# payakorn/InteriorPointMethod

Hardware: AMD Instinct MI355X
Metric: IPM iterations/sec (m=4096,n=8192 dense LP) (higher is better)
Workload: dtype f64; 1 GPU; dense synthetic LP m=4096 n=8192 fp64, seed 0, start x=s=1 y=0 (BASELINE.json configs[1]); replicas per GPU

## Files before the change

interiorpointmethod_amd/csrc/ipm_api.hip:

```cpp
#include <hip/hip_runtime.h>
#include <hip/hip_ext.h>
#include <math.h>
#include <stdarg.h>
#include <stdio.h>
#include <stdlib.h>
#include <string.h>

#include <deque>
#include <vector>

#include "../../include/ipm_hip.h"
#include "gemm_nt_f64.h"
#include "adat_syrk_f64.h"
#include "chol_update_f64.h"
#include "potrf_f64.h"
#include "sparse_ops.h"
#include "trsv_grouped.h"
#include "getrf_f64.h"
#include "small_lp.h"
#include "sparse_chol.h"
#include "sparse_symbolic.h"
#include "vector_ops.h"
#include "form_factor.h"
#include "lockstep.h"
#include "lockstep_merge.h"

#include <algorithm>
#include <atomic>
#include <mutex>
#include <chrono>
#include <limits>
#include <utility>

using namespace ipm;

static thread_local char g_err[512] = "";

static const int MAX_DEVICES = 64;
static std::atomic<int> g_live[MAX_DEVICES];
static std::atomic<bool> g_attr_set[MAX_DEVICES];

struct ipm_handle {
    int device = 0;
    hipStream_t stream = nullptr;
    bool own_stream = false;
    hipStream_t stream2 = nullptr;
    hipStream_t stream3 = nullptr;
    hipEvent_t ev_mid = nullptr, ev_res = nullptr, ev_grp = nullptr, ev_last = nullptr;
    std::vector<hipEvent_t> ev_diag, ev_crit, ev_bulk;
    hipEvent_t ev_fork = nullptr;
    int lookahead = 1;
    int grouped_trsv = 1;
    int gsz = 0;
    double *gXT = nullptr, *gX = nullptr, *gS = nullptr, *gPart = nullptr;
    unsigned* d_bulk_done = nullptr;
    bool no_dense = false;
    double* B_own = nullptr; double* invD_own = nullptr;
    int group_steps = 0;
    int two_level = 1;
    int bulk_variant = 0;
    int ss_small_blocks = 16;
    int flag_sync = 1;
    int last_gs = 1, n_counter_steps = 0, n_event_steps = 0, timeouts_recovered = 0;
    bool counted = false;
    bool small = false;
    int fused_small = 1;
    bool list_form = false;
    int list_form_opt = 1;
    int *ls_bi = nullptr, *ls_bk = nullptr;
    double* ls_bak = nullptr;
    int sm_nb = 0;
    int *sm_bptr = nullptr, *sm_bcol = nullptr;
    unsigned short *sm_bi = nullptr, *sm_bk = nullptr;
    double* sm_bcoef = nullptr;
    bool spf = false;
    bool spf_off = false;
    bool sp_serial = false;
    SpFactor spF;
    std::vector<void*> sp_allocs;
    int *sp_fptr = nullptr, *sp_fcol = nullptr;
    double* sp_fcoef = nullptr;
    long long* sp_diagpos = nullptr;
    long long sp_nslot = 0, sp_nu = 0, sp_terms = 0;
    int sp_height = 0, sp_rmax = 0, sp_grid = 1, sp_serial_launches = 0, sp_nvirtual = 0;
    size_t sp_lds_chol = 0, sp_lds_solve = 0;
    int sp_fv_off = 0;
    int sp_fuse_fwd = 1;
    const double* sp_fwd_fused = nullptr;
    int sp_lds_doubles = 16, sp_threads = 256;
    int sp_level_mode = 0;
    std::vector<int> sp_lvlptr;
    SpRec* sp_rec_level = nullptr;
    unsigned sp_epoch = 0;
    double shift_rel = 0.0;
    int auto_reg = 0;
    unsigned* d_flags = nullptr;
    int64_t m = 0, n = 0, mp = 0, np = 0;
    int nblk = 0, rc_chunks = 0, rows_per_chunk = 0, vblk = 0;
    ipm_options opt;
    void* ws = nullptr;
    size_t ws_bytes = 0;
    bool own_ws = false;
    double *A = nullptr, *B = nullptr, *invD = nullptr;
    double *x = nullptr, *s = nullptr, *c = nullptr, *rc = nullptr, *d = nullptr, *v = nullptr, *q = nullptr;
    double *dxa = nullptr, *dsa = nullptr, *dx = nullptr, *ds = nullptr;
    double *y = nullptr, *b = nullptr, *rb = nullptr, *t1 = nullptr, *t2 = nullptr, *dya = nullptr, *dy = nullptr;
    double *atp = nullptr, *part = nullptr, *slab = nullptr;
    int ff_enabled = 1;
    int ff_min_nblk = 16, ff_max_nblk = 72;
    bool ff_forced = false;
    int ff_chain_mode = 1;
    int ff_q = 4;
    int ff_workers = 0;
    int* d_ff_tile_items = nullptr;
    int ff_qmax = 16;
    bool ff_built = false, ff_last = false;
    FFSchedule ff_sched;
    FFItem* d_ff_items = nullptr;
    unsigned* d_ff_flags = nullptr;
    size_t ff_flag_words = 0;
    double* ff_slab = nullptr;
    double* ff_part = nullptr;
    hipEvent_t ev_ffjoin = nullptr;
    long long* ff_trace = nullptr;
    long long* ff_prof = nullptr;
    const int* fdone = nullptr;
    std::vector<int> env_last, env_first;
    bool use_env = false;
    int envelope = 1;
    bool sparse = false;
    int64_t nnz_cap = 0, nnz = 0;
    int* d_tile_order = nullptr;
    int *d_rowptr = nullptr, *d_colind = nullptr, *d_colptr = nullptr, *d_rowind = nullptr;
    double *d_rval = nullptr, *d_cval = nullptr;
    long long* stamp_buf = nullptr;
    unsigned* ff_potrfdone = nullptr;
    Scalars* sc = nullptr;
    IterRec* hist = nullptr;
    double* snap = nullptr;
    bool bnd = false;
    int bnd_nU = 0;
    double* bnd_mem = nullptr;
    bool detect = false;
    double det_eps_p = 1e-8, det_eps_d = 1e-8;
    double* det = nullptr;
    double* cert_mem = nullptr;
    int* fixed = nullptr;
    Scalars* h_sc = nullptr;
    bool haveA = false, haveBC = false, haveState = false, predictor_valid = false;
    bool fresh_state = true;
    int profiling = 0;
    double phase_ms[4] = {0, 0, 0, 0};
    hipEvent_t ev0 = nullptr, ev1 = nullptr;
// ... 280 lines not shown
    if (const char* e = getenv("IPM_ENVELOPE")) h->envelope = atoi(e);
    CREATE_TRY(hipMemsetAsync(base + L.off_inv, 0, L.off_slab - L.off_inv, h->stream));
    {
        std::lock_guard<std::mutex> lock(g_hsc_mutex);
        if (!g_hsc_pool.empty()) { h->h_sc = g_hsc_pool.back(); g_hsc_pool.pop_back(); }
    }
    if (!h->h_sc) CREATE_TRY(hipHostMalloc((void**)&h->h_sc, sizeof(Scalars), hipHostMallocDefault));
    memset(h->h_sc, 0, sizeof(Scalars));
    CREATE_TRY(hipEventCreate(&h->ev0));
    CREATE_TRY(hipEventCreate(&h->ev1));
    if (const char* e = getenv("IPM_LOOKAHEAD")) h->lookahead = atoi(e);
    h->detect = (h->opt.flags & IPM_FLAG_DETECT_INFEASIBILITY) != 0;
    if (h->opt.flags & IPM_FLAG_LOCKSTEP) { h->lockstep = 1; h->opt.flags |= IPM_FLAG_SINGLE_STREAM | IPM_FLAG_NO_DEVICE_POLLING; }
    if (h->opt.flags & IPM_FLAG_SINGLE_STREAM) h->lookahead = 0;
    if (const char* e = getenv("IPM_GROUPED_TRSV")) h->grouped_trsv = atoi(e);
    if (h->lockstep && getenv("IPM_LS_BLOCK_STEPS")) h->grouped_trsv = 0;
    if (h->lockstep) h->ss_small_blocks = 1 << 20;
    if (h->no_dense) h->grouped_trsv = 0;
    h->gsz = 0;
    if (h->grouped_trsv) {
        const bool ragged = !(getenv("IPM_RAGGED_GROUPS") && atoi(getenv("IPM_RAGGED_GROUPS")) == 0);
        if (h->nblk >= 2 * GS_MAX) { if (ragged || h->nblk % GS_MAX == 0) h->gsz = GS_MAX; }
        else {
            for (int p2 = GS_MAX; p2 >= 2; p2 /= 2) if (h->nblk % p2 == 0) { h->gsz = p2; break; }
            if (ragged && h->nblk > GS_MAX && h->gsz < 4) h->gsz = GS_MAX;
        }
    }
    if (h->gsz > 0) {
        const size_t nG = (size_t)h->nblk / h->gsz, GR = (size_t)h->gsz * 128;
        CREATE_TRY(dev_malloc(device, h->stream, (void**)&h->gXT, sizeof(double) * nG * GR * GR));
        CREATE_TRY(dev_malloc(device, h->stream, (void**)&h->gX, sizeof(double) * nG * GR * GR));
        CREATE_TRY(dev_malloc(device, h->stream, (void**)&h->gS, sizeof(double) * nG * (GR / 2) * (GR / 2)));
        CREATE_TRY(dev_malloc(device, h->stream, (void**)&h->gPart, sizeof(double) * 16 * (size_t)h->mp));
        CREATE_TRY(hipMemsetAsync(h->gXT, 0, sizeof(double) * nG * GR * GR, h->stream));
        CREATE_TRY(hipMemsetAsync(h->gX, 0, sizeof(double) * nG * GR * GR, h->stream));
    } else {
        h->grouped_trsv = 0;
    }
    CREATE_TRY(dev_malloc(device, h->stream, (void**)&h->d_flags, sizeof(unsigned) * (2 * (size_t)h->nblk + 4)));
    CREATE_TRY(hipMemsetAsync(h->d_flags, 0, sizeof(unsigned) * (2 * (size_t)h->nblk + 4), h->stream));
    CREATE_TRY(dev_malloc(device, h->stream, (void**)&h->d_bulk_done, sizeof(unsigned) * (2 * (size_t)h->nblk + 4)));
    CREATE_TRY(hipMemsetAsync(h->d_bulk_done, 0, sizeof(unsigned) * (2 * (size_t)h->nblk + 4), h->stream));
    if (const char* e = getenv("IPM_FLAG_SYNC")) h->flag_sync = atoi(e);
    if (h->opt.flags & IPM_FLAG_NO_DEVICE_POLLING) h->flag_sync = 0;
    if (const char* e = getenv("IPM_BULK_VARIANT")) h->bulk_variant = atoi(e);
    if (const char* e = getenv("IPM_TWO_LEVEL")) h->two_level = atoi(e);
    if (const char* e = getenv("IPM_GROUP_STEPS")) h->group_steps = atoi(e);
    if (const char* e = getenv("IPM_FUSED_SMALL")) h->fused_small = atoi(e);
    if (const char* e = getenv("IPM_LIST_FORM")) h->list_form_opt = atoi(e);
    if (getenv("IPM_POTRF_STAMPS")) { CREATE_TRY(dev_malloc(device, h->stream, (void**)&h->stamp_buf, 8 * 64 * sizeof(long long))); CREATE_TRY(hipMemsetAsync(h->stamp_buf, 0, 8 * 64 * sizeof(long long), h->stream)); }
    if (h->lookahead != 0 && h->nblk > 2)
        CREATE_TRY(hipStreamCreateWithFlags(&h->stream2, hipStreamNonBlocking));
    CREATE_TRY(hipEventCreateWithFlags(&h->ev_fork, hipEventDisableTiming));
    if (!h->sparse && h->lookahead != 0 && h->nblk >= 16)
        CREATE_TRY(hipStreamCreateWithFlags(&h->stream3, hipStreamNonBlocking));
    CREATE_TRY(hipEventCreateWithFlags(&h->ev_mid, hipEventDisableTiming));
    CREATE_TRY(hipEventCreateWithFlags(&h->ev_res, hipEventDisableTiming));
    CREATE_TRY(hipEventCreateWithFlags(&h->ev_grp, hipEventDisableTiming));
    CREATE_TRY(hipEventCreateWithFlags(&h->ev_last, hipEventDisableTiming));
    if (const char* e = getenv("IPM_FUSED_FACTOR")) { if (!strcmp(e, "force")) { h->ff_enabled = 1; h->ff_min_nblk = 3; h->ff_forced = true; } else h->ff_enabled = atoi(e); }
    if (const char* e = getenv("IPM_FF_MAX_NBLK")) h->ff_max_nblk = atoi(e);
    if (const char* e = getenv("IPM_FF_CHAIN_MODE")) {
        if (atoi(e) == 0) {
            int rc_ = fail(nullptr, IPM_ERR_INVALID_ARG, "IPM_FF_CHAIN_MODE=0 is not supported (the fused launch runs chain mode 1 only)");
            ipm_destroy(h);
            return rc_;
        }
    }
    if (const char* e = getenv("IPM_FF_Q")) h->ff_q = std::max(1, std::min(16, atoi(e)));
    CREATE_TRY(hipEventCreateWithFlags(&h->ev_ffjoin, hipEventDisableTiming));
    h->ev_diag.assign(h->nblk, nullptr); h->ev_crit.assign(h->nblk, nullptr); h->ev_bulk.assign(h->nblk, nullptr);
    for (int k = 0; k < h->nblk; ++k) {
        CREATE_TRY(hipEventCreateWithFlags(&h->ev_diag[k], hipEventDisableTiming));
        CREATE_TRY(hipEventCreateWithFlags(&h->ev_crit[k], hipEventDisableTiming));
        CREATE_TRY(hipEventCreateWithFlags(&h->ev_bulk[k], hipEventDisableTiming));
    }
    if (h->sparse && h->mp <= SP_LDS_MAX_MP && device < MAX_DEVICES && !g_attr_set[device].load(std::memory_order_acquire)) {
        CREATE_TRY(hipFuncSetAttribute((const void*)adat_sparse_kernel, hipFuncAttributeMaxDynamicSharedMemorySize, SP_LDS_MAX_MP * 8));
        g_attr_set[device].store(true, std::memory_order_release);
    }
    hipLaunchKernelGGL(set_params_kernel, dim3(1), dim3(1), 0, h->stream, h->sc, 1e-8, 1e-8, 1e-8, h->opt.eta, 5000, 0, 1);
    CREATE_TRY(hipGetLastError());
// ... 4 lines not shown
    return IPM_OK;
}

extern "C" int ipm_destroy(ipm_handle* h) {
    if (!h) return IPM_OK;
    (void)hipSetDevice(h->device);
    if (h->ff_prof) {
        (void)hipDeviceSynchronize();
        std::vector<long long> P(16 * ((size_t)h->ff_workers + 1));
        (void)hipMemcpy(P.data(), h->ff_prof, sizeof(long long) * P.size(), hipMemcpyDeviceToHost);
        double tot[16] = {0};
        for (int w = 0; w <= h->ff_workers; ++w) for (int k = 0; k < 16; ++k) tot[k] += (double)P[(size_t)w * 16 + k];
        static const char* nm[] = {"ticket", "F gemm", "F store+publish", "T wait", "T gemm", "T base+combine", "panel wait", "panel gemm", "T store+publish"};
        double sum = 0; for (int k = 0; k < 9; ++k) sum += tot[k];
        fprintf(stderr, "[ff prof] %d workers, F items %.0f, T items %.0f, cycles per worker in the launches %.3g (sum of phases %.3g)\n", h->ff_workers, tot[FFP_NF], tot[FFP_NT], tot[FFP_TOTAL] / h->ff_workers, sum / h->ff_workers);
        for (int k = 0; k < 9; ++k) fprintf(stderr, "   %-18s %6.2f %%\n", nm[k], 100.0 * tot[k] / sum);
    }
    if (h->counted) g_live[h->device].fetch_sub(1, std::memory_order_acq_rel);
    if (h->stream) (void)hipStreamSynchronize(h->stream);
    if (h->stream2) (void)hipStreamSynchronize(h->stream2);
    for (auto& v : {&h->ev_diag, &h->ev_crit, &h->ev_bulk})
        for (hipEvent_t e : *v) if (e) (void)hipEventDestroy(e);
    if (h->ev_fork) (void)hipEventDestroy(h->ev_fork);
    if (h->stream3) { (void)hipStreamSynchronize(h->stream3); (void)hipStreamDestroy(h->stream3); }
    if (h->ev_mid) (void)hipEventDestroy(h->ev_mid);
    if (h->ev_res) (void)hipEventDestroy(h->ev_res);
    if (h->ev_grp) (void)hipEventDestroy(h->ev_grp);
    if (h->ev_last) (void)hipEventDestroy(h->ev_last);
    if (h->ev_ffjoin) (void)hipEventDestroy(h->ev_ffjoin);
    if (h->stream2) (void)hipStreamDestroy(h->stream2);
    if (h->ev0) (void)hipEventDestroy(h->ev0);
    if (h->ev1) (void)hipEventDestroy(h->ev1);
    if (h->h_sc) { std::lock_guard<std::mutex> lock(g_hsc_mutex); g_hsc_pool.push_back(h->h_sc); h->h_sc = nullptr; }
    for (void* p : {(void*)h->stamp_buf, (void*)h->d_flags, (void*)h->d_bulk_done, (void*)h->B_own, (void*)h->invD_own, (void*)h->bnd_mem, (void*)h->cert_mem, (void*)h->gXT, (void*)h->gX, (void*)h->gS, (void*)h->gPart})
        dev_free(h->device, h->stream, p);
    ff_release(h);
    free_sparse_factor(h);
    for (void* p : {(void*)h->sm_bptr, (void*)h->sm_bcol, (void*)h->sm_bi, (void*)h->sm_bk, (void*)h->sm_bcoef, (void*)h->ls_bi, (void*)h->ls_bk, (void*)h->ls_bak})
        dev_free(h->device, h->stream, p);
    if (h->own_ws && h->ws) (void)hipFree(h->ws);
    if (h->own_stream && h->stream) (void)hipStreamDestroy(h->stream);
    delete h;
    return IPM_OK;
}

static bool all_finite(const double* p, int64_t rows, int64_t cols, int64_t ld) {
    for (int64_t i = 0; i < rows; ++i)
        for (int64_t j = 0; j < cols; ++j)
            if (!isfinite(p[i * ld + j])) return false;
    return true;
}

extern "C" int ipm_set_A_dense(ipm_handle* h, const double* A, int64_t ld, int is_device) {
    if (!h || !A || ld < h->n) return fail(h, IPM_ERR_INVALID_ARG, "ipm_set_A_dense: bad arguments");
    if (h->sparse) return fail(h, IPM_ERR_STATE, "ipm_set_A_dense: the handle was created for a sparse A (sparse_nnz > 0)");
    HIP_TRY(h, hipSetDevice(h->device));
    if (!is_device && !all_finite(A, h->m, h->n, ld)) return fail(h, IPM_ERR_INVALID_INPUT, "A has non-finite entries");
    HIP_TRY(h, hipMemsetAsync(h->A, 0, sizeof(double) * h->mp * h->np, h->stream));
    HIP_TRY(h, hipMemcpy2DAsync(h->A, sizeof(double) * h->np, A, sizeof(double) * ld, sizeof(double) * h->n, h->m,
                                is_device ? hipMemcpyDeviceToDevice : hipMemcpyHostToDevice, h->stream));
    HIP_TRY(h, hipStreamSynchronize(h->stream));
    h->haveA = true; h->predictor_valid = false;
    return IPM_OK;
}

static void free_sparse_factor(ipm_handle* h) {
    for (void* p : h->sp_allocs) dev_free(h->device, h->stream, p);
// ... 924 lines not shown
    h->ff_qmax = 1;
    for (int q_ : h->ff_sched.tile_q) h->ff_qmax = std::max(h->ff_qmax, q_);
    if (nstages > 65535) return fail(h, IPM_ERR_INVALID_ARG, "fused factor: %d formation stages exceed the 16-bit stage range of a work item", nstages);
    const size_t ntile = (size_t)h->nblk * (h->nblk + 1) / 2;
    {
        std::vector<int> fcnt(ntile, 0), base(ntile, 0), applied(ntile, 0), paneled(ntile, 0);
        for (const FFItem& it : h->ff_sched.items) {
            const size_t t = (size_t)ff_tile(it.i, it.c);
            if (it.type == FF_D) continue;
            if (it.type == FF_F) {
                if (it.c <= it.i) fcnt[t]++;
                if (it.i + 1 < h->nblk) fcnt[(size_t)ff_tile(it.i + 1, it.c)]++;
                continue;
            }
            if (it.t.j0 != applied[t]) return fail(h, IPM_ERR_INVALID_ARG, "fused factor: internal error (column order of tile %d,%d)", it.i, it.c);
            applied[t] = it.t.j1;
            if (it.t.flags & FF_ADD_BASE) base[t]++;
            if (it.t.flags & FF_PANEL) paneled[t]++;
        }
        for (int i = 0; i < h->nblk; ++i)
            for (int c = 0; c <= i; ++c) {
                const size_t t = (size_t)ff_tile(i, c);
                if (fcnt[t] != h->ff_sched.tile_q[t] || base[t] != 1 || applied[t] != ff_limit(i, c) || paneled[t] != (ff_needs_panel(i, c) ? 1 : 0))
                    return fail(h, IPM_ERR_INVALID_ARG, "fused factor: internal error (tile %d,%d incomplete in the work list)", i, c);
            }
    }
    const size_t nit = h->ff_sched.items.size();
    HIP_TRY(h, dev_malloc(h->device, h->stream, (void**)&h->d_ff_items, sizeof(FFItem) * nit));
    HIP_TRY(h, hipMemcpyAsync(h->d_ff_items, h->ff_sched.items.data(), sizeof(FFItem) * nit, hipMemcpyHostToDevice, h->stream));
    HIP_TRY(h, dev_malloc(h->device, h->stream, (void**)&h->d_ff_tile_items, sizeof(int) * 2 * ntile));
    HIP_TRY(h, hipMemcpyAsync(h->d_ff_tile_items, h->ff_sched.tile_items.data(), sizeof(int) * ntile, hipMemcpyHostToDevice, h->stream));
    HIP_TRY(h, hipMemcpyAsync(h->d_ff_tile_items + ntile, h->ff_sched.tile_q.data(), sizeof(int) * ntile, hipMemcpyHostToDevice, h->stream));
    h->ff_flag_words = 32 + 2 * ntile + 3 * (size_t)h->nblk;
    HIP_TRY(h, dev_malloc(h->device, h->stream, (void**)&h->d_ff_flags, sizeof(unsigned) * 2 * h->ff_flag_words));
    HIP_TRY(h, dev_malloc(h->device, h->stream, (void**)&h->ff_slab, sizeof(double) * ntile * (size_t)h->ff_qmax * 128 * 128));
    HIP_TRY(h, dev_malloc(h->device, h->stream, (void**)&h->ff_part, sizeof(double) * 256));
    if (getenv("IPM_FF_PROF")) {
        HIP_TRY(h, dev_malloc(h->device, h->stream, (void**)&h->ff_prof, sizeof(long long) * 16 * ((size_t)h->ff_workers + 1)));
        HIP_TRY(h, hipMemsetAsync(h->ff_prof, 0, sizeof(long long) * 16 * ((size_t)h->ff_workers + 1), h->stream));
    }
    if (getenv("IPM_FF_TRACE_ITEMS")) {
        const size_t words = 4 * nit + 12 * (size_t)h->nblk;
        HIP_TRY(h, dev_malloc(h->device, h->stream, (void**)&h->ff_trace, sizeof(long long) * words));
        HIP_TRY(h, hipMemsetAsync(h->ff_trace, 0, sizeof(long long) * words, h->stream));
    }
    HIP_TRY(h, hipStreamSynchronize(h->stream));
    h->ff_built = true;
    return IPM_OK;
}

static void ff_release(ipm_handle* h) {
    for (void** p : {(void**)&h->d_ff_items, (void**)&h->d_ff_flags, (void**)&h->ff_slab, (void**)&h->ff_part, (void**)&h->ff_prof, (void**)&h->ff_trace,
                     (void**)&h->d_ff_tile_items}) { dev_free(h->device, h->stream, *p); *p = nullptr; }
    h->ff_built = false;
}
static bool ff_use(ipm_handle* h) {
    if (!ff_ok(h)) return false;
    if (h->ff_built) return true;
    if (ff_build(h) == IPM_OK) return true;
    ff_release(h);
    h->ff_enabled = 0;
    (void)hipGetLastError();
    return false;
}

static int enqueue_form_factor(ipm_handle* h, hipEvent_t* ev, int mid_step, int ginv_step) {
    if (!h->ff_built) return fail(h, IPM_ERR_STATE, "fused factor: schedule not built");
    const int nblk = h->nblk;
    const size_t ntile = (size_t)nblk * (nblk + 1) / 2;
    const int* done = h->fdone ? h->fdone : &h->sc->done;
    hipStream_t sw = h->stream, sm = h->stream2;
    unsigned* F = h->d_ff_flags;
    unsigned *ticket = F, *mticket = F + 16, *dbg = F + 24, *fcount = F + 32, *tprog = fcount + ntile, *lfinal = tprog + ntile, *dready = lfinal + nblk,
             *potrfdone = dready + nblk;
    unsigned* timeout = h->d_flags + 2 * (size_t)nblk;
    h->ff_potrfdone = potrfdone;
    HIP_TRY(h, hipMemsetAsync(F, 0, sizeof(unsigned) * h->ff_flag_words, sw));
    HIP_TRY(h, hipEventRecord(h->ev_fork, sw));
    if (!h->ff_chain_mode) HIP_TRY(h, hipStreamWaitEvent(sm, h->ev_fork, 0));
    long long* ctrace = h->ff_trace ? h->ff_trace + 4 * h->ff_sched.items.size() : nullptr;
    FFRoles roles;
    memset(&roles, 0, sizeof roles);
    if (h->ff_chain_mode) {
        FFChain& c = roles.chain;
        c.B = h->B; c.ldb = h->mp; c.invD = h->invD;
        c.maxbits = (const unsigned long long*)(F + 8); c.dcount = F + 10; c.maxdiag_out = &h->sc->maxdiag;
        c.dready = dready; c.potrfdone = potrfdone; c.timeout = timeout; c.dbg = dbg; c.trace = ctrace;
        c.eps = h->opt.pivot_guard_eps; c.big = h->opt.pivot_guard_big; c.shift_rel = h->shift_rel;
        c.fixed = &h->sc->fixed; c.done = done; c.nblk = nblk; c.m = (int)h->m;
        FFCrit& cc = roles.crit;
        cc.B = h->B; cc.ldb = h->mp; cc.invD = h->invD; cc.tprog = tprog; cc.tile_items = h->d_ff_tile_items;
        cc.potrfdone = potrfdone; cc.lfinal = lfinal; cc.dready = dready; cc.timeout = timeout; cc.dbg = dbg; cc.trace = ctrace;
        cc.done = done; cc.nblk = nblk;
        roles.role = F + 3;
    } else {
        hipLaunchKernelGGL(ff_maxdiag_kernel, dim3(256), dim3(256), 0, sm, h->A, h->np, (int)h->m, (int)h->np, h->d, h->ff_part, mticket,
                           &h->sc->maxdiag, done);
    }
    FFArgs a;
    memset(&a, 0, sizeof a);
    a.A = h->A; a.lda = h->np; a.d = h->d; a.B = h->B; a.ldb = h->mp; a.invD = h->invD; a.slab = h->ff_slab;
    a.items = h->d_ff_items; a.nitems = (int)h->ff_sched.items.size();
    a.ticket = ticket; a.fcount = fcount; a.tprog = tprog; a.lfinal = lfinal; a.dready = dready; a.potrfdone = potrfdone;
    a.timeout = timeout; a.dbg = dbg; a.done = done;
    { static const bool dbg_on = getenv("IPM_FF_DEBUG") != nullptr; a.dbg_words = dbg_on ? (unsigned)h->ff_flag_words : 0u; }
    a.trace = h->ff_trace;
    a.prof = h->ff_prof;
    a.tile_q = h->d_ff_tile_items + ntile;
    a.maxbits = (unsigned long long*)(F + 8); a.dcount = F + 10;
    a.nblk = nblk; a.Q = h->ff_qmax; a.nstages = (int)(h->np / FF_PBK); a.m = (int)h->m;
    if (ev) HIP_TRY(h, hipEventRecord(ev[1], sw));
    {
        if (h->ff_chain_mode) {
            const dim3 grid((unsigned)h->ff_workers + 1u + (unsigned)FF_CRIT_WGS);
            if (a.prof || a.trace) hipLaunchKernelGGL((form_factor_roles_kernel<true>), grid, dim3(FF_THREADS), 0, sw, a, roles);
            else hipLaunchKernelGGL((form_factor_roles_kernel<false>), grid, dim3(FF_THREADS), 0, sw, a, roles);
        } else {
            const dim3 grid((unsigned)h->ff_workers);
            if (a.prof || a.trace) hipLaunchKernelGGL((form_factor_kernel<true>), grid, dim3(FF_THREADS), 0, sw, a);
            else hipLaunchKernelGGL((form_factor_kernel<false>), grid, dim3(FF_THREADS), 0, sw, a);
        }
    }
    if (ev) HIP_TRY(h, hipEventRecord(ev[2], sw));
    HIP_TRY(h, hipGetLastError());
    h->n_counter_steps = 0; h->n_event_steps = 0; h->last_gs = 1;
    if (h->ff_chain_mode) {
        h->n_counter_steps = nblk;
        const int gate_step = ginv_step >= 0 ? ginv_step : mid_step;
        if (gate_step >= 0) {
            HIP_TRY(h, hipStreamWaitEvent(h->stream3, h->ev_fork, 0));
            hipLaunchKernelGGL(ff_gate_kernel, dim3(1), dim3(64), 0, h->stream3, potrfdone + gate_step, 1u, timeout, done);
            if (ginv_step >= 0) { int rc_ = enqueue_group_inverses(h, 0, (ginv_step + 1) / h->gsz, h->stream3); if (rc_) return rc_; }
            if (mid_step >= 0) {
                int rc_ = enqueue_residuals(h, h->stream3);
                if (rc_) return rc_;
                launch_gemv_n(h, h->v, -1.0, -1.0, h->rb, h->t1, h->stream3);
                HIP_TRY(h, hipEventRecord(h->ev_res, h->stream3));
            }
        }
        HIP_TRY(h, hipGetLastError());
        h->ff_last = true;
        return IPM_OK;
    }
    for (int k = 0; k < nblk; ++k) {
        PotrfDiag pd;
        pd.Bkk = h->B + (int64_t)k * NB * (h->mp + 1); pd.ld = h->mp;
        pd.inv = h->invD + (int64_t)k * NB * NB;
        pd.maxdiag = &h->sc->maxdiag; pd.eps = h->opt.pivot_guard_eps; pd.big = h->opt.pivot_guard_big; pd.shift_rel = h->shift_rel;
        pd.fixed = &h->sc->fixed; pd.done = done; pd.stamps = nullptr;
        pd.wait_on = dready + k; pd.wait_count = 10; pd.signal = potrfdone + k; pd.timeout = timeout; pd.dbg = dbg; pd.dbg_tag = (unsigned)k;
        pd.trace = ctrace ? ctrace + 12 * (size_t)k : nullptr;
        pd.nt = potrf_panels(h, k);
        pd.rows = (int)(h->m - (int64_t)k * NB);
        hipLaunchKernelGGL(potrf_diag_kernel<false>, dim3(1), dim3(PD_THREADS), 0, sm, pd);
        ++h->n_counter_steps;
        if (k == ginv_step) {
            HIP_TRY(h, hipEventRecord(h->ev_grp, sm));
            HIP_TRY(h, hipStreamWaitEvent(h->stream3, h->ev_grp, 0));
            int rc_ = enqueue_group_inverses(h, 0, (k + 1) / h->gsz, h->stream3);
            if (rc_) return rc_;
        }
        if (k == mid_step) { int rc_ = enqueue_residual_stream(h, sm); if (rc_) return rc_; }
        if (k + 1 >= nblk) break;
// ... 127 lines not shown
        launch_dense_gemv_n(h, h->gX + (int64_t)g * GR * GR, GR, GR, GR, r + (int64_t)g * GR, 1.0, 0.0, nullptr, z + (int64_t)g * GR);
        int below = (int)(h->mp - (int64_t)(g + 1) * GR);
        if (h->use_env) below = std::min(below, (int)((int64_t)(h->env_last[(g + 1) * GS - 1] + 1) * NB - (int64_t)(g + 1) * GR));
        if (below > 0) {
            double* rb = r + (int64_t)(g + 1) * GR;
            launch_dense_gemv_n(h, h->B + (int64_t)(g + 1) * GR * h->mp + (int64_t)g * GR, h->mp, below, GR, z + (int64_t)g * GR, -1.0, 1.0,
                                rb, rb);
        }
    }
    const int k_left = nG * GS;
    if (k_left < h->nblk) {
        TrsvStep a;
        a.L = h->B; a.ld = h->mp; a.inv = h->invD; a.done = done;
        a.r = r; a.z = z; a.j0 = 0;
        for (int k = k_left; k < h->nblk; ++k) {
            a.k = k;
            const int nb = h->use_env ? h->env_last[k] - k + 1 : h->nblk - k;
            if (!ls_push(h, LS_TRSV_FWD, (unsigned)nb, a)) hipLaunchKernelGGL(trsv_fwd_step_kernel, dim3(nb), dim3(256), 0, h->stream, a);
        }
        a.r = z; a.z = out;
        for (int k = h->nblk - 1; k >= k_left; --k) {
            a.k = k;
            a.j0 = h->use_env ? h->env_first[k] : 0;
            if (!ls_push(h, LS_TRSV_BWD, (unsigned)(k - a.j0 + 1), a)) hipLaunchKernelGGL(trsv_bwd_step_kernel, dim3(k - a.j0 + 1), dim3(256), 0, h->stream, a);
        }
    }
    for (int g = nG - 1; g >= 0; --g) {
        launch_dense_gemv_n(h, h->gXT + (int64_t)g * GR * GR, GR, GR, GR, z + (int64_t)g * GR, 1.0, 0.0, nullptr, out + (int64_t)g * GR);
        int left = g * GR;
        const int c0 = h->use_env ? std::min(left, h->env_first[g * GS] * NB) : 0;
        left -= c0;
        if (left > 0) {
            dim3 grid((unsigned)((left + 511) / 512), 16);
            if (!ls_push(h, LS_GEMV_T, grid.x * 16u, LsGemvT{h->B + (int64_t)g * GR * h->mp + c0, h->mp, GR / 16, left, out + (int64_t)g * GR, h->gPart, done, grid.x}))
                hipLaunchKernelGGL(gemv_t_kernel, grid, dim3(256), 0, h->stream, h->B + (int64_t)g * GR * h->mp + c0, h->mp, GR / 16, left,
                                   out + (int64_t)g * GR, h->gPart, done);
            if (!ls_push(h, LS_SUB_PARTIALS, (unsigned)((left + 255) / 256), LsSubPart{z + c0, h->gPart, left, 16, done}))
                hipLaunchKernelGGL(sub_partials_kernel, dim3((unsigned)((left + 255) / 256)), dim3(256), 0, h->stream, z + c0, h->gPart, left, 16, done);
        }
    }
    HIP_TRY(h, hipGetLastError());
    return IPM_OK;
}

static int enqueue_potrs(ipm_handle* h, double* r, double* out, hipEvent_t wait_last = nullptr) {
    if (sp_on(h)) {
        const int rm = std::max(16, h->sp_rmax);
#define SP_LAUNCH_FWD(NT, SC, GRID, RECS, COUNT) \
    hipLaunchKernelGGL((sp_fwd_kernel<NT, SC>), dim3(GRID), dim3(NT), h->sp_lds_solve, h->stream, h->spF, ep, r, h->t2, rm, RECS, COUNT)
#define SP_LAUNCH_BWD(NT, SC, GRID, RECS, COUNT) \
    hipLaunchKernelGGL((sp_bwd_kernel<NT, SC>), dim3(GRID), dim3(NT), 0, h->stream, h->spF, ep, h->t2, out, RECS, COUNT)
#define SP_SWEEP(WHICH, GRID, RECS, COUNT)                                                                                            \
    do {                                                                                                                             \
        WHICH(SPC_THREADS, false, GRID, RECS, COUNT);                                                                                \
    } while (0)
        unsigned ep = ++h->sp_epoch;
        const size_t nlev = h->sp_lvlptr.size() > 0 ? h->sp_lvlptr.size() - 1 : 0;
        const bool fwd_done = h->sp_fwd_fused != nullptr && h->sp_fwd_fused == r;
        h->sp_fwd_fused = nullptr;
        if (sp_level(h)) {
            for (size_t l = 0; l < nlev && !fwd_done; ++l) {
                const int cnt = h->sp_lvlptr[l + 1] - h->sp_lvlptr[l];
                SP_SWEEP(SP_LAUNCH_FWD, (unsigned)std::min(cnt, h->sp_grid), h->sp_rec_level + h->sp_lvlptr[l], cnt);
            }
            for (size_t l = nlev; l-- > 0;) {
                const int cnt = h->sp_lvlptr[l + 1] - h->sp_lvlptr[l];
// ... 78 lines not shown

static int enqueue_iteration(ipm_handle* h, hipEvent_t* ev) {
    int rc;
    const bool all = ev && h->profiling >= 2;
    if (overlap_residuals(h)) {
        VecArgs a = vec_args(h);
        if (h->bnd) hipLaunchKernelGGL(scaling_bounded_kernel, dim3(h->vblk), dim3(VBLK), 0, h->stream, a, bnd_args(h));
        else hipLaunchKernelGGL(scaling_kernel, dim3(h->vblk), dim3(VBLK), 0, h->stream, a);
        const bool fused = ff_use(h);
        if (ev && !fused) HIP_TRY(h, hipEventRecord(ev[1], h->stream));
        struct Latch { ipm_handle* h; ~Latch() { h->fdone = nullptr; } } latch{h};
        h->fdone = &h->sc->done_f;
        h->ff_last = false;
        if (!fused) {
            if ((rc = enqueue_form(h, h->d))) return rc;
            if (ev) HIP_TRY(h, hipEventRecord(ev[2], h->stream));
        }
        const int rstep = h->nblk * 13 / 16;
        const int nG = h->grouped_trsv ? h->nblk / h->gsz : 0;
        const int gstep = (nG >= 2 && (nG - 1) * h->gsz - 1 < rstep) ? (nG - 1) * h->gsz - 1 : -1;
        if (fused) { if ((rc = enqueue_form_factor(h, ev, rstep, gstep))) return rc; }
        else if ((rc = enqueue_factor(h, true, rstep, gstep))) return rc;
        h->fdone = nullptr;
        if (gstep >= 0) {
            if (h->ff_last && h->ff_chain_mode && h->ff_potrfdone) {
                hipLaunchKernelGGL(ff_gate_kernel, dim3(1), dim3(64), 0, h->stream3, h->ff_potrfdone + (h->nblk - 1), 1u, h->d_flags + 2 * (size_t)h->nblk, &h->sc->done);
            } else {
                HIP_TRY(h, hipEventRecord(h->ev_grp, h->stream));
                HIP_TRY(h, hipStreamWaitEvent(h->stream3, h->ev_grp, 0));
            }
            if ((rc = enqueue_group_inverses(h, nG - 1, nG, h->stream3))) return rc;
            HIP_TRY(h, hipEventRecord(h->ev_last, h->stream3));
            HIP_TRY(h, hipStreamWaitEvent(h->stream, h->ev_res, 0));
            if ((rc = enqueue_predictor(h, nullptr, true, h->ev_last))) return rc;
        } else {
            if ((rc = enqueue_group_inverses(h, 0, nG, nullptr))) return rc;
            HIP_TRY(h, hipStreamWaitEvent(h->stream, h->ev_res, 0));
            if ((rc = enqueue_predictor(h, nullptr, true))) return rc;
        }
        if ((rc = enqueue_corrector(h, nullptr))) return rc;
        if ((rc = enqueue_update(h))) return rc;
        return IPM_OK;
    }
    if (all) HIP_TRY(h, hipEventRecord(ev[0], h->stream));
    if ((rc = enqueue_residuals(h))) return rc;
    h->ff_last = false;
    bool have_rhs = false;
    if (h->profiling < 2 && ff_use(h)) {
        if ((rc = enqueue_form_factor(h, ev, -1, -1))) return rc;
    } else {
        if (ev) HIP_TRY(h, hipEventRecord(ev[1], h->stream));
        if ((rc = enqueue_form(h, h->d))) return rc;
        if (ev) HIP_TRY(h, hipEventRecord(ev[2], h->stream));
        if (sp_on(h) && h->sp_fuse_fwd) {
            launch_gemv_n(h, h->v, -1.0, -1.0, h->rb, h->t1);
            have_rhs = true;
            if ((rc = enqueue_factor(h, true, -1, -1, h->t1))) return rc;
        } else if ((rc = enqueue_factor(h, true))) return rc;
    }
    if ((rc = enqueue_group_inverses(h))) return rc;
    if (all) HIP_TRY(h, hipEventRecord(ev[3], h->stream));
    if ((rc = enqueue_predictor(h, all ? ev + 4 : nullptr, have_rhs))) return rc;
    if ((rc = enqueue_corrector(h, all ? ev + 6 : nullptr))) return rc;
    if ((rc = enqueue_update(h))) return rc;
    if (all) HIP_TRY(h, hipEventRecord(ev[8], h->stream));
    return IPM_OK;
}

static int read_scalars(ipm_handle* h, bool* timed_out = nullptr) {
    unsigned tmo = 0;
    unsigned* word = h->d_flags + 2 * (size_t)h->nblk;
    HIP_TRY(h, hipMemcpyAsync(h->h_sc, h->sc, sizeof(Scalars), hipMemcpyDeviceToHost, h->stream));
    HIP_TRY(h, hipMemcpyAsync(&tmo, word, sizeof(unsigned), hipMemcpyDeviceToHost, h->stream));
    HIP_TRY(h, hipStreamSynchronize(h->stream));
    if (tmo) {
        if (h->stream2) HIP_TRY(h, hipStreamSynchronize(h->stream2));
        if (h->ff_built && h->ff_last && getenv("IPM_FF_DEBUG")) {
            std::vector<unsigned> F(h->ff_flag_words);
            (void)hipMemcpy(F.data(), h->d_ff_flags, sizeof(unsigned) * F.size(), hipMemcpyDeviceToHost);
            if (F[24] && F[26] < 6) {
                std::vector<unsigned> S(h->ff_flag_words);
                (void)hipMemcpy(S.data(), h->d_ff_flags + h->ff_flag_words, sizeof(unsigned) * S.size(), hipMemcpyDeviceToHost);
                for (size_t w = 0; w < F.size(); ++w) if (w < 24 || w >= 32) F[w] = S[w];
                fprintf(stderr, "[ff debug] (snapshot taken by the first wait that gave up)\n");
            }
            const int nb = h->nblk; const size_t nt = (size_t)nb * (nb + 1) / 2;
            const unsigned *fc = F.data() + 32, *tp = fc + nt, *lf = tp + nt, *dr = lf + nb, *pd = dr + nb;
            fprintf(stderr, "[ff debug] ticket %u of %zu items; first worker wait that gave up: count %u item %u kind %u target %u seen %u\n", F[0],
                    h->ff_sched.items.size(), F[24], F[25], F[26], F[27], F[28]);
            if (F[24] && F[26] < 6 && F[25] < h->ff_sched.items.size()) {
                const FFItem& it = h->ff_sched.items[F[25]];
                fprintf(stderr, "  that item: T(%d,%d)[%d,%d) flags %d seq %d\n", it.i, it.c, it.t.j0, it.t.j1, it.t.flags, it.t.seq);
            }
            fprintf(stderr, "  potrfdone:");
            for (int k = 0; k < nb; ++k) fprintf(stderr, " %u", pd[k]);
            fprintf(stderr, "\n  dready:");
            for (int k = 0; k < nb; ++k) fprintf(stderr, " %u", dr[k]);
            fprintf(stderr, "\n  lfinal:");
            for (int k = 0; k < nb; ++k) fprintf(stderr, " %u", lf[k]);
            fprintf(stderr, "\n  incomplete tiles (i,c: fcount/expected tprog/expected):");
            int shown = 0;
            for (int i = 0; i < nb; ++i)
                for (int c = 0; c <= i; ++c) {
                    const size_t t = (size_t)ff_tile(i, c);
                    if ((fc[t] != (unsigned)h->ff_sched.tile_q[t] || tp[t] != (unsigned)h->ff_sched.tile_items[t]) && shown++ < 24)
                        fprintf(stderr, " (%d,%d: %u/%d %u/%d)", i, c, fc[t], h->ff_sched.tile_q[t], tp[t], h->ff_sched.tile_items[t]);
                }
            fprintf(stderr, "\n");
        }
        HIP_TRY(h, hipMemsetAsync(word, 0, sizeof(unsigned), h->stream));
        if (!timed_out) return fail(h, IPM_ERR_HIP, "a device-side hand-off poll timed out (persistent solve)");
    }
    if (timed_out) *timed_out = tmo != 0;
    return IPM_OK;
}

static void poll_fallback(ipm_handle* h) {
    if (h->spf) h->sp_serial = true;
    if (h->ff_last) h->ff_enabled = 0;
    else h->flag_sync = 0;
    ++h->timeouts_recovered;
}

__global__ __launch_bounds__(256) void snapshot_kernel(double* x, double* y, double* s, Scalars* sc, double* snap, int np,
                                                       int mp, int restore) {
    const int gid = blockIdx.x * 256 + threadIdx.x, gsz = gridDim.x * 256;
    double *sx = snap, *ss = snap + np, *sy = snap + 2 * (size_t)np;
    Scalars* ssc = (Scalars*)(snap + 2 * (size_t)np + mp);
    if (restore) {
        for (int j = gid; j < np; j += gsz) { x[j] = sx[j]; s[j] = ss[j]; }
        for (int i = gid; i < mp; i += gsz) y[i] = sy[i];
        if (gid == 0) *sc = *ssc;
    } else {
        for (int j = gid; j < np; j += gsz) { sx[j] = x[j]; ss[j] = s[j]; }
        for (int i = gid; i < mp; i += gsz) sy[i] = y[i];
        if (gid == 0) *ssc = *sc;
    }
}
__global__ __launch_bounds__(256) void snapshot_bounds_kernel(double* w, double* z, double* sw, double* sz, int np, int restore) {
    const int gid = blockIdx.x * 256 + threadIdx.x, gsz = gridDim.x * 256;
    for (int j = gid; j < np; j += gsz) {
        if (restore) { w[j] = sw[j]; z[j] = sz[j]; }
        else { sw[j] = w[j]; sz[j] = z[j]; }
    }
}
static int enqueue_snapshot(ipm_handle* h, int restore, hipStream_t st = nullptr) {
    const int64_t mx = h->np > h->mp ? h->np : h->mp;
    const unsigned grid = (unsigned)std::min<int64_t>((mx + 255) / 256, 256);
    hipLaunchKernelGGL(snapshot_kernel, dim3(grid), dim3(256), 0, st ? st : h->stream, h->x, h->y, h->s, h->sc, h->snap, (int)h->np,
                       (int)h->mp, restore);
// ... 871 lines not shown
```

interiorpointmethod_amd/csrc/trsv_grouped.h:

```cpp
#pragma once
#include <hip/hip_runtime.h>
#include <stdint.h>
#include "gemm_nt_f64.h"

namespace ipm {

constexpr int GS_MAX = 8;

__device__ __forceinline__ void group_diag_transpose_kernel_body(const double* __restrict__ invD, double* XT, double* X, int b0, int GS, const int* done,
                                                                  const unsigned bx_, const unsigned by_, const unsigned bz_) {
    if (done && *done) return;
    __shared__ double tile[32][33];
    const int64_t GR = (int64_t)GS * 128;
    const int b = b0 + bz_, g = b / GS, a = b % GS;
    const double* src = invD + (int64_t)b * 128 * 128;
    double* dst = XT + (int64_t)g * GR * GR + (int64_t)(a * 128) * GR + a * 128;
    double* dsx = X + (int64_t)g * GR * GR + (int64_t)(a * 128) * GR + a * 128;
    const int bx = bx_ * 32, by = by_ * 32;
    for (int j = threadIdx.y; j < 32; j += 8) {
        double v = src[(int64_t)(by + j) * 128 + bx + threadIdx.x];
        tile[j][threadIdx.x] = v;
        dsx[(int64_t)(by + j) * GR + bx + threadIdx.x] = v;
    }
    __syncthreads();
    for (int j = threadIdx.y; j < 32; j += 8) dst[(int64_t)(bx + j) * GR + by + threadIdx.x] = tile[threadIdx.x][j];
}
__global__ void group_diag_transpose_kernel(const double* __restrict__ invD, double* XT, double* X, int b0, int GS, const int* done) {
    group_diag_transpose_kernel_body(invD, XT, X, b0, GS, done, blockIdx.x, blockIdx.y, blockIdx.z);
}

__device__ __forceinline__ void sub_partials_kernel_body(double* z, const double* __restrict__ part, int np, int rc,
                                                           const int* done, const unsigned bx_, const unsigned gx_) {
    if (done && *done) return;
    const int c = bx_ * 256 + threadIdx.x;
    if (c >= np) return;
    double s = 0.0;
    int r = 0;
    for (; r + 8 <= rc; r += 8) {
        double t[8];
#pragma unroll
        for (int q = 0; q < 8; ++q) t[q] = part[(int64_t)(r + q) * np + c];
#pragma unroll
        for (int q = 0; q < 8; ++q) s += t[q];
    }
    for (; r < rc; ++r) s += part[(int64_t)r * np + c];
    z[c] -= s;
}
__global__ __launch_bounds__(256) void sub_partials_kernel(double* z, const double* __restrict__ part, int np, int rc,
                                                           const int* done) { sub_partials_kernel_body(z, part, np, rc, done, blockIdx.x, gridDim.x); }

}
```

Baseline: 260.2 iterations/s.

## Fuse gemv_t with partial-sum reduction via tickets and double-buffer fused-factor flags

Adds a gemv_t_sub kernel where the last block per column chunk, found through an atomic ticket counter, reduces the partials into z. This removes the separate sub_partials launch in the grouped triangular solve tail. The fused-factor flag array is also double-buffered so the next solve's flag zeroing can run early on stream3 instead of as a memset on the critical stream. This adds atomic and fence ordering complexity and a risk of stale flags if the zeroed-set bookkeeping goes wrong.

```diff
diff --git a/interiorpointmethod_amd/csrc/ipm_api.hip b/interiorpointmethod_amd/csrc/ipm_api.hip
--- a/interiorpointmethod_amd/csrc/ipm_api.hip
+++ b/interiorpointmethod_amd/csrc/ipm_api.hip
@@ -53,6 +53,8 @@
     int grouped_trsv = 1;
     int gsz = 0;
     double *gXT = nullptr, *gX = nullptr, *gS = nullptr, *gPart = nullptr;
+    unsigned* gTicket = nullptr;
+    int tail_overlap = 1;
     unsigned* d_bulk_done = nullptr;
     bool no_dense = false;
     double* B_own = nullptr; double* invD_own = nullptr;
@@ -119,6 +121,10 @@
     FFItem* d_ff_items = nullptr;
     unsigned* d_ff_flags = nullptr;
     size_t ff_flag_words = 0;
+    unsigned* ff_F = nullptr;
+    int ff_set = 0;
+    bool ff_zeroed[2] = {false, false};
+    int ff_zero_pending = -1;
     double* ff_slab = nullptr;
     double* ff_part = nullptr;
     hipEvent_t ev_ffjoin = nullptr;
@@ -465,6 +471,8 @@
         CREATE_TRY(dev_malloc(device, h->stream, (void**)&h->gX, sizeof(double) * nG * GR * GR));
         CREATE_TRY(dev_malloc(device, h->stream, (void**)&h->gS, sizeof(double) * nG * (GR / 2) * (GR / 2)));
         CREATE_TRY(dev_malloc(device, h->stream, (void**)&h->gPart, sizeof(double) * 16 * (size_t)h->mp));
+        CREATE_TRY(dev_malloc(device, h->stream, (void**)&h->gTicket, sizeof(unsigned) * (((size_t)h->mp + 511) / 512)));
+        CREATE_TRY(hipMemsetAsync(h->gTicket, 0, sizeof(unsigned) * (((size_t)h->mp + 511) / 512), h->stream));
         CREATE_TRY(hipMemsetAsync(h->gXT, 0, sizeof(double) * nG * GR * GR, h->stream));
         CREATE_TRY(hipMemsetAsync(h->gX, 0, sizeof(double) * nG * GR * GR, h->stream));
     } else {
@@ -481,6 +489,7 @@
     if (const char* e = getenv("IPM_GROUP_STEPS")) h->group_steps = atoi(e);
     if (const char* e = getenv("IPM_FUSED_SMALL")) h->fused_small = atoi(e);
     if (const char* e = getenv("IPM_LIST_FORM")) h->list_form_opt = atoi(e);
+    if (const char* e = getenv("IPM_TAIL_OVERLAP")) h->tail_overlap = atoi(e);
     if (getenv("IPM_POTRF_STAMPS")) { CREATE_TRY(dev_malloc(device, h->stream, (void**)&h->stamp_buf, 8 * 64 * sizeof(long long))); CREATE_TRY(hipMemsetAsync(h->stamp_buf, 0, 8 * 64 * sizeof(long long), h->stream)); }
     if (h->lookahead != 0 && h->nblk > 2)
         CREATE_TRY(hipStreamCreateWithFlags(&h->stream2, hipStreamNonBlocking));
@@ -551,7 +560,7 @@
     if (h->ev0) (void)hipEventDestroy(h->ev0);
     if (h->ev1) (void)hipEventDestroy(h->ev1);
     if (h->h_sc) { std::lock_guard<std::mutex> lock(g_hsc_mutex); g_hsc_pool.push_back(h->h_sc); h->h_sc = nullptr; }
-    for (void* p : {(void*)h->stamp_buf, (void*)h->d_flags, (void*)h->d_bulk_done, (void*)h->B_own, (void*)h->invD_own, (void*)h->bnd_mem, (void*)h->cert_mem, (void*)h->gXT, (void*)h->gX, (void*)h->gS, (void*)h->gPart})
+    for (void* p : {(void*)h->stamp_buf, (void*)h->d_flags, (void*)h->d_bulk_done, (void*)h->B_own, (void*)h->invD_own, (void*)h->bnd_mem, (void*)h->cert_mem, (void*)h->gXT, (void*)h->gX, (void*)h->gS, (void*)h->gPart, (void*)h->gTicket})
         dev_free(h->device, h->stream, p);
     ff_release(h);
     free_sparse_factor(h);
@@ -1542,7 +1551,8 @@
     HIP_TRY(h, hipMemcpyAsync(h->d_ff_tile_items, h->ff_sched.tile_items.data(), sizeof(int) * ntile, hipMemcpyHostToDevice, h->stream));
     HIP_TRY(h, hipMemcpyAsync(h->d_ff_tile_items + ntile, h->ff_sched.tile_q.data(), sizeof(int) * ntile, hipMemcpyHostToDevice, h->stream));
     h->ff_flag_words = 32 + 2 * ntile + 3 * (size_t)h->nblk;
-    HIP_TRY(h, dev_malloc(h->device, h->stream, (void**)&h->d_ff_flags, sizeof(unsigned) * 2 * h->ff_flag_words));
+    HIP_TRY(h, dev_malloc(h->device, h->stream, (void**)&h->d_ff_flags, sizeof(unsigned) * 4 * h->ff_flag_words));
+    h->ff_set = 0; h->ff_zeroed[0] = h->ff_zeroed[1] = false; h->ff_zero_pending = -1; h->ff_F = h->d_ff_flags;
     HIP_TRY(h, dev_malloc(h->device, h->stream, (void**)&h->ff_slab, sizeof(double) * ntile * (size_t)h->ff_qmax * 128 * 128));
     HIP_TRY(h, dev_malloc(h->device, h->stream, (void**)&h->ff_part, sizeof(double) * 256));
     if (getenv("IPM_FF_PROF")) {
@@ -1563,6 +1573,7 @@
     for (void** p : {(void**)&h->d_ff_items, (void**)&h->d_ff_flags, (void**)&h->ff_slab, (void**)&h->ff_part, (void**)&h->ff_prof, (void**)&h->ff_trace,
                      (void**)&h->d_ff_tile_items}) { dev_free(h->device, h->stream, *p); *p = nullptr; }
     h->ff_built = false;
+    h->ff_F = nullptr; h->ff_zeroed[0] = h->ff_zeroed[1] = false; h->ff_zero_pending = -1;
 }
 static bool ff_use(ipm_handle* h) {
     if (!ff_ok(h)) return false;
@@ -1580,12 +1591,17 @@
     const size_t ntile = (size_t)nblk * (nblk + 1) / 2;
     const int* done = h->fdone ? h->fdone : &h->sc->done;
     hipStream_t sw = h->stream, sm = h->stream2;
-    unsigned* F = h->d_ff_flags;
+    const int set = h->ff_set;
+    unsigned* F = h->d_ff_flags + (size_t)set * 2 * h->ff_flag_words;
+    h->ff_F = F;
+    h->ff_set = h->tail_overlap ? set ^ 1 : set;
+    h->ff_zero_pending = -1;
     unsigned *ticket = F, *mticket = F + 16, *dbg = F + 24, *fcount = F + 32, *tprog = fcount + ntile, *lfinal = tprog + ntile, *dready = lfinal + nblk,
              *potrfdone = dready + nblk;
     unsigned* timeout = h->d_flags + 2 * (size_t)nblk;
     h->ff_potrfdone = potrfdone;
-    HIP_TRY(h, hipMemsetAsync(F, 0, sizeof(unsigned) * h->ff_flag_words, sw));
+    if (!h->ff_zeroed[set]) HIP_TRY(h, hipMemsetAsync(F, 0, sizeof(unsigned) * h->ff_flag_words, sw));
+    h->ff_zeroed[set] = false;
     HIP_TRY(h, hipEventRecord(h->ev_fork, sw));
     if (!h->ff_chain_mode) HIP_TRY(h, hipStreamWaitEvent(sm, h->ev_fork, 0));
     long long* ctrace = h->ff_trace ? h->ff_trace + 4 * h->ff_sched.items.size() : nullptr;
@@ -1639,6 +1655,11 @@
         const int gate_step = ginv_step >= 0 ? ginv_step : mid_step;
         if (gate_step >= 0) {
             HIP_TRY(h, hipStreamWaitEvent(h->stream3, h->ev_fork, 0));
+            if (h->tail_overlap && mid_step >= 0) {
+                const int nx = set ^ 1;
+                HIP_TRY(h, hipMemsetAsync(h->d_ff_flags + (size_t)nx * 2 * h->ff_flag_words, 0, sizeof(unsigned) * h->ff_flag_words, h->stream3));
+                h->ff_zero_pending = nx;
+            }
             hipLaunchKernelGGL(ff_gate_kernel, dim3(1), dim3(64), 0, h->stream3, potrfdone + gate_step, 1u, timeout, done);
             if (ginv_step >= 0) { int rc_ = enqueue_group_inverses(h, 0, (ginv_step + 1) / h->gsz, h->stream3); if (rc_) return rc_; }
             if (mid_step >= 0) {
@@ -1832,6 +1853,11 @@
         left -= c0;
         if (left > 0) {
             dim3 grid((unsigned)((left + 511) / 512), 16);
+            if (h->tail_overlap && !h->ls_rec) {
+                hipLaunchKernelGGL(gemv_t_sub_kernel, grid, dim3(256), 0, h->stream, h->B + (int64_t)g * GR * h->mp + c0, h->mp, GR / 16,
+                                   left, out + (int64_t)g * GR, h->gPart, z + c0, h->gTicket, done);
+                continue;
+            }
             if (!ls_push(h, LS_GEMV_T, grid.x * 16u, LsGemvT{h->B + (int64_t)g * GR * h->mp + c0, h->mp, GR / 16, left, out + (int64_t)g * GR, h->gPart, done, grid.x}))
                 hipLaunchKernelGGL(gemv_t_kernel, grid, dim3(256), 0, h->stream, h->B + (int64_t)g * GR * h->mp + c0, h->mp, GR / 16, left,
                                    out + (int64_t)g * GR, h->gPart, done);
@@ -1976,10 +2002,12 @@
             if ((rc = enqueue_group_inverses(h, nG - 1, nG, h->stream3))) return rc;
             HIP_TRY(h, hipEventRecord(h->ev_last, h->stream3));
             HIP_TRY(h, hipStreamWaitEvent(h->stream, h->ev_res, 0));
+            if (h->ff_zero_pending >= 0) { h->ff_zeroed[h->ff_zero_pending] = true; h->ff_zero_pending = -1; }
             if ((rc = enqueue_predictor(h, nullptr, true, h->ev_last))) return rc;
         } else {
             if ((rc = enqueue_group_inverses(h, 0, nG, nullptr))) return rc;
             HIP_TRY(h, hipStreamWaitEvent(h->stream, h->ev_res, 0));
+            if (h->ff_zero_pending >= 0) { h->ff_zeroed[h->ff_zero_pending] = true; h->ff_zero_pending = -1; }
             if ((rc = enqueue_predictor(h, nullptr, true))) return rc;
         }
         if ((rc = enqueue_corrector(h, nullptr))) return rc;
@@ -2021,10 +2049,10 @@
         if (h->stream2) HIP_TRY(h, hipStreamSynchronize(h->stream2));
         if (h->ff_built && h->ff_last && getenv("IPM_FF_DEBUG")) {
             std::vector<unsigned> F(h->ff_flag_words);
-            (void)hipMemcpy(F.data(), h->d_ff_flags, sizeof(unsigned) * F.size(), hipMemcpyDeviceToHost);
+            (void)hipMemcpy(F.data(), h->ff_F, sizeof(unsigned) * F.size(), hipMemcpyDeviceToHost);
             if (F[24] && F[26] < 6) {
                 std::vector<unsigned> S(h->ff_flag_words);
-                (void)hipMemcpy(S.data(), h->d_ff_flags + h->ff_flag_words, sizeof(unsigned) * S.size(), hipMemcpyDeviceToHost);
+                (void)hipMemcpy(S.data(), h->ff_F + h->ff_flag_words, sizeof(unsigned) * S.size(), hipMemcpyDeviceToHost);
                 for (size_t w = 0; w < F.size(); ++w) if (w < 24 || w >= 32) F[w] = S[w];
                 fprintf(stderr, "[ff debug] (snapshot taken by the first wait that gave up)\n");
             }
@@ -2060,6 +2088,7 @@
 }
 
 static void poll_fallback(ipm_handle* h) {
+    h->ff_zeroed[0] = h->ff_zeroed[1] = false;
     if (h->spf) h->sp_serial = true;
     if (h->ff_last) h->ff_enabled = 0;
     else h->flag_sync = 0;
diff --git a/interiorpointmethod_amd/csrc/trsv_grouped.h b/interiorpointmethod_amd/csrc/trsv_grouped.h
--- a/interiorpointmethod_amd/csrc/trsv_grouped.h
+++ b/interiorpointmethod_amd/csrc/trsv_grouped.h
@@ -2,6 +2,7 @@
 #include <hip/hip_runtime.h>
 #include <stdint.h>
 #include "gemm_nt_f64.h"
+#include "vector_ops.h"
 
 namespace ipm {
 
@@ -49,4 +50,28 @@
 __global__ __launch_bounds__(256) void sub_partials_kernel(double* z, const double* __restrict__ part, int np, int rc,
                                                            const int* done) { sub_partials_kernel_body(z, part, np, rc, done, blockIdx.x, gridDim.x); }
 
+__global__ __launch_bounds__(256) void gemv_t_sub_kernel(const double* __restrict__ A, int64_t lda, int rows_per_chunk, int np,
+                                                         const double* __restrict__ u, double* part, double* z, unsigned* ticket,
+                                                         const int* done) {
+    __shared__ unsigned last_s;
+    const bool skip = done && *done;
+    if (!skip) gemv_t_kernel_body(A, lda, rows_per_chunk, np, u, part, nullptr, blockIdx.x, blockIdx.y);
+    asm volatile("s_waitcnt vmcnt(0)" ::: "memory");
+    __syncthreads();
+    if (threadIdx.x == 0) {
+        __builtin_amdgcn_fence(__ATOMIC_RELEASE, "agent");
+        asm volatile("s_waitcnt vmcnt(0)" ::: "memory");
+        const unsigned t = __hip_atomic_fetch_add(ticket + blockIdx.x, 1u, __ATOMIC_RELAXED, __HIP_MEMORY_SCOPE_AGENT);
+        last_s = (t & (gridDim.y - 1)) == gridDim.y - 1 ? 1u : 0u;
+        if (last_s) {
+            __builtin_amdgcn_fence(__ATOMIC_ACQUIRE, "agent");
+            asm volatile("s_waitcnt vmcnt(0)" ::: "memory");
+        }
+    }
+    __syncthreads();
+    if (!last_s || skip) return;
+    sub_partials_kernel_body(z, part, np, (int)gridDim.y, nullptr, blockIdx.x * 2, 0);
+    sub_partials_kernel_body(z, part, np, (int)gridDim.y, nullptr, blockIdx.x * 2 + 1, 0);
 }
+
+}
```

After: 263.4 iterations/s (median of 6 runs). +1.2%, better.
